# line/Human-Interaction-Generation

Measured on AMD Instinct MI355X. Metric: denoiser-fwd frames/s @ B=64·T=196, higher is better.
Workload: dtype f32; 1 GPU; MotionTransformer forward incl. the per-call cross-attention text side, BASELINE config 2: B=64/GPU T=196 F=150 d=512 L=8 H=8 ff=1024 N=77 Lt=256, linear attention, text embeddings supplied (CLIP stubbed); parallelism=dp1

## Files before the change

### human-interaction-generation_amd/csrc/linattn.hip

```cpp
#include <stdlib.h>

#include "hig_host.h"

namespace {

constexpr int CH = 64;

template <int HD> struct Patch {
  static constexpr int PC = HD >= 128 ? 8 : HD >= 64 ? 4 : HD >= 32 ? 2 : 1;
  static constexpr int PL = PC;
  static constexpr int TL = HD / PL;
};

template <int HD>
__global__ __launch_bounds__(256) void ctx_kernel(const float* __restrict__ K,
                                                  const float* __restrict__ V, int64_t ld, int rows,
                                                  int H, const int64_t* __restrict__ length,
                                                  float* __restrict__ A, float* __restrict__ kstat) {
  constexpr int LDP = HD + 4;
  constexpr int PC = Patch<HD>::PC, PL = Patch<HD>::PL, TL = Patch<HD>::TL;
  constexpr int RG = 256 / HD;
  __shared__ __attribute__((aligned(16))) float sP[CH * LDP];
  __shared__ __attribute__((aligned(16))) float sV[CH * LDP];
  __shared__ float sred[256];
// ... 1388 lines not shown
template <class F> void with_mfma_hd(int hd, F&& f) {
  if (hd == 64) f(std::integral_constant<int, 64>{});
  else f(std::integral_constant<int, 128>{});
}
#define HDC(c) decltype(c)::value

template <typename T> uintptr_t row_bits(int64_t ld) { return hig_low_bits(ld, (int)sizeof(T)); }
template <typename T, class... P> uintptr_t row_bits(int64_t ld, const void* p, P... more) { return hig_low_bits(p) | row_bits<T>(ld, more...); }

}

extern "C" int64_t hig_linattn_ctx_scratch_floats(int32_t B, int32_t rows, int32_t H, int32_t hd) {
  const int64_t nchunk = (rows + CH - 1) / CH;
  return (int64_t)B * H * nchunk * ((int64_t)hd * hd + 2 * hd);
}

namespace {
template <typename TIO>
int launch_ctx(const hig_attn_plan_t& p, const TIO* K, const TIO* V, int64_t ld, int32_t B, int32_t rows, int32_t H, int32_t hd,
               const int64_t* length, float* A, float* kstat, float* scratch, __bf16* At16, hipStream_t st) {
  with_mfma_hd(hd, [&](auto c) {
    if (p.path == HIG_ATTN_PATH_CTX_PART) {
      hipLaunchKernelGGL((ctx_part_mfma_kernel<HDC(c), TIO>), dim3(B * H, p.split), dim3(256), 0, st, K, V, ld, rows, H, length, scratch);
      hipLaunchKernelGGL(ctx_combine_kernel<HDC(c)>, dim3(B * H), dim3(256), 0, st, scratch, p.split, A, kstat, At16);
    } else {
      hipLaunchKernelGGL((ctx_mfma_kernel<HDC(c), TIO>), dim3(B * H), dim3(256), 0, st, K, V, ld, rows, H, length, A, kstat, At16, CtxGroups{H, 0, 0});
    }
  });
  HIG_CHECK_LAUNCH();
  return HIG_OK;
}

template <typename TIO>
int launch_apply(const hig_attn_plan_t& p, const TIO* Q, int64_t ldq, const float* A, TIO* Y, int64_t ldy, int32_t B, int32_t rows, int32_t H,
                 int32_t hd, hipStream_t st) {
  if constexpr (sizeof(TIO) == 4) {
    if (p.path == HIG_ATTN_PATH_APPLY_WAVE64) {
      hipLaunchKernelGGL(apply_wave64_kernel, dim3(B * H), dim3(256), 0, st, reinterpret_cast<const float*>(Q), ldq, A,
                         reinterpret_cast<float*>(Y), ldy, rows, H);
      HIG_CHECK_LAUNCH();
      return HIG_OK;
    }
  }
  with_mfma_hd(hd, [&](auto c) {
    hipLaunchKernelGGL((apply_mfma_kernel<HDC(c), TIO>), dim3(B * H, p.split), dim3(256), 0, st, Q, ldq, A, Y, ldy, rows, H);
  });
  HIG_CHECK_LAUNCH();
  return HIG_OK;
}
}

extern "C" int hig_linattn_ctx(const float* K, const float* V, int64_t ld, int32_t B, int32_t rows,
                               int32_t H, int32_t hd, const int64_t* length, float* A, float* kstat,
                               float* scratch, hig_stream_t stream) {
  hig_attn_plan_t p;
  HIG_TRY(hig_attn_plan_entry(&p, {HIG_ATTN_ENTRY_CTX, HIG_ATTN_IO_F32, B, rows, 0, H, hd, scratch != nullptr, hig_attn_facts(K && V && A && kstat, 0, 0)}));
  if (p.path != HIG_ATTN_PATH_CTX) return launch_ctx<float>(p, K, V, ld, B, rows, H, hd, length, A, kstat, scratch, nullptr, hig_stream(stream));
  HD_SWITCH(hd, hipLaunchKernelGGL((ctx_kernel<HDV>), dim3(B * H), dim3(256), 0, hig_stream(stream), K, V,
                                   ld, rows, H, length, A, kstat));
  HIG_CHECK_LAUNCH();
  return HIG_OK;
}

int hig_linattn_ctx_groups(const float* K, const float* V, int64_t ld, int32_t B, int32_t rows, int32_t H, int32_t G, int32_t hd,
                           float* A, int64_t a_gs, float* kstat, int64_t k_gs, hipStream_t st) {
  if (!hig_attn_mfma_hd(hd) || B <= 0 || rows <= 0 || H <= 0 || G <= 0) return 1;
  with_mfma_hd(hd, [&](auto c) {
    hipLaunchKernelGGL((ctx_mfma_kernel<HDC(c), float>), dim3(B * H * G), dim3(256), 0, st, K, V, ld, rows, H * G, nullptr, A, kstat, nullptr,
                       CtxGroups{H, a_gs, k_gs});
  });
  hig_attn_path_count(HIG_ATTN_PATH_CTX_MFMA, 1);
  HIG_CHECK_LAUNCH();
  return HIG_OK;
}

extern "C" int hig_linattn_apply(const float* Q, int64_t ldq, const float* A, float* Y, int64_t ldy,
                                 int32_t B, int32_t rows, int32_t H, int32_t hd, hig_stream_t stream) {
  hig_attn_plan_t p;
  HIG_TRY(hig_attn_plan_entry(&p, {HIG_ATTN_ENTRY_APPLY, HIG_ATTN_IO_F32, B, rows, 0, H, hd, false,
                     hig_attn_facts(Q && A && Y, row_bits<float>(ldq, Q), row_bits<float>(ldy, Y))}));
  if (p.path != HIG_ATTN_PATH_APPLY) return launch_apply<float>(p, Q, ldq, A, Y, ldy, B, rows, H, hd, hig_stream(stream));
  HD_SWITCH(hd, hipLaunchKernelGGL((apply_kernel<HDV>), dim3(B * H, p.split), dim3(256), 0, hig_stream(stream), Q, ldq, A, Y, ldy, rows, H));
  HIG_CHECK_LAUNCH();
  return HIG_OK;
}

namespace {

template <typename TO> __device__ __forceinline__ float apply_sty_act(float x) { return hig_silu_fast(x); }
template <> __device__ __forceinline__ float apply_sty_act<float>(float x) { return hig_silu(x); }

template <typename T> struct Vec16 {};
template <> struct Vec16<float> { static constexpr int N = 4; };
template <> struct Vec16<__bf16> { static constexpr int N = 8; };
typedef unsigned u32x4_t __attribute__((ext_vector_type(4)));
typedef float f32x4_t __attribute__((ext_vector_type(4)));
__device__ __forceinline__ void put16(float* dst, u32x4_t raw, const float*) {
  *reinterpret_cast<u32x4_t*>(dst) = raw;
}
__device__ __forceinline__ void put16(float* dst, u32x4_t raw, const __bf16*) {
  *reinterpret_cast<f32x4_t*>(dst) = f32x4_t{__uint_as_float(raw.x << 16), __uint_as_float(raw.x & 0xffff0000u),
                                             __uint_as_float(raw.y << 16), __uint_as_float(raw.y & 0xffff0000u)};
  *reinterpret_cast<f32x4_t*>(dst + 4) = f32x4_t{__uint_as_float(raw.z << 16), __uint_as_float(raw.z & 0xffff0000u),
                                                 __uint_as_float(raw.w << 16), __uint_as_float(raw.w & 0xffff0000u)};
}

template <int HD, typename TQ, typename TO>
__global__ __launch_bounds__(256) void apply_sty_kernel(const TQ* __restrict__ Q, int64_t ldq,
                                                        const float* __restrict__ A, const float* __restrict__ gamma,
                                                        const float* __restrict__ beta, const float* __restrict__ ss,
                                                        int64_t ss_ld, int shift_off, TO* __restrict__ Out,
                                                        int64_t ldo, int rows, int H, int nblk) {
  constexpr int TB = HD / 32;
  constexpr int KC = 4096 / HD;
  constexpr int NSLAB = HD / KC;
  constexpr int MAXHPW = 2;
  constexpr int QLD = HD + 4;
  constexpr int EQ = Vec16<TQ>::N;
  constexpr int CPR = HD / EQ;
  constexpr int NQL = 32 * CPR / 64;
  extern __shared__ __attribute__((aligned(16))) char smem_dyn[];
  __shared__ float red[2][4][32];
  const int tid = threadIdx.x, lane = tid & 63, wave = tid >> 6;
  const int lr = lane & 31, kk = lane >> 5;
  const int b = blockIdx.x / nblk, r0 = (blockIdx.x % nblk) * 32;
  const int HPW = H / 4;
  const int d = H * HD;
  constexpr int WBUF = 32 * QLD > KC * HD ? 32 * QLD : KC * HD;
  float* sAw = reinterpret_cast<float*>(smem_dyn) + wave * WBUF;
  float* sQw = sAw;

  f32x16 acc[MAXHPW][TB];
#pragma unroll
  for (int hh = 0; hh < MAXHPW; ++hh)
#pragma unroll
    for (int tb = 0; tb < TB; ++tb) zero16(acc[hh][tb]);

  u32x4_t pq[NQL];
  f32x4_t pa[16];
  auto fetch_q = [&](int h) {
#pragma unroll
    for (int i = 0; i < NQL; ++i) {
      const int idx = lane + 64 * i, rr = idx / CPR, c = idx % CPR;
      const int row = min(r0 + rr, rows - 1);
      pq[i] = *reinterpret_cast<const u32x4_t*>(Q + ((int64_t)b * rows + row) * ldq + h * HD + EQ * c);
    }
  };
  auto fetch_a = [&](int h, int c0) {
    const f32x4_t* src = reinterpret_cast<const f32x4_t*>(A + (((int64_t)b * H + h) * HD + c0) * HD);
#pragma unroll
    for (int i = 0; i < 16; ++i) pa[i] = src[lane + 64 * i];
  };
  fetch_q(wave * HPW);
  fetch_a(wave * HPW, 0);

#pragma unroll
  for (int hh = 0; hh < MAXHPW; ++hh) {
    if (hh >= HPW) break;
    const int h = wave * HPW + hh;
#pragma unroll
    for (int i = 0; i < NQL; ++i) {
      const int idx = lane + 64 * i, rr = idx / CPR, c = idx % CPR;
      put16(sQw + rr * QLD + EQ * c, pq[i], static_cast<const TQ*>(nullptr));
    }
    if (hh + 1 < HPW) fetch_q(h + 1);
    f32x4_t q[HD / 8];
    float m = -INFINITY;
#pragma unroll
    for (int ks = 0; ks < HD / 8; ++ks) {
      q[ks] = *reinterpret_cast<const f32x4_t*>(sQw + lr * QLD + 8 * ks + 4 * kk);
      m = fmaxf(m, fmaxf(fmaxf(q[ks].x, q[ks].y), fmaxf(q[ks].z, q[ks].w)));
    }
    m = fmaxf(m, __shfl_xor(m, 32, 64));
    float sum = 0.f;
#pragma unroll
    for (int ks = 0; ks < HD / 8; ++ks) {
      q[ks].x = __expf(q[ks].x - m); q[ks].y = __expf(q[ks].y - m); q[ks].z = __expf(q[ks].z - m); q[ks].w = __expf(q[ks].w - m);
      sum += (q[ks].x + q[ks].y) + (q[ks].z + q[ks].w);
    }
    sum += __shfl_xor(sum, 32, 64);
    const float inv = 1.0f / sum;
#pragma unroll
    for (int ks = 0; ks < HD / 8; ++ks) q[ks] *= inv;
#pragma unroll
    for (int sl = 0; sl < NSLAB; ++sl) {
      const int c0 = sl * KC;
#pragma unroll
      for (int i = 0; i < 16; ++i) reinterpret_cast<f32x4_t*>(sAw)[lane + 64 * i] = pa[i];
      if (sl + 1 < NSLAB) fetch_a(h, c0 + KC);
      else if (hh + 1 < HPW) fetch_a(h + 1, 0);
#pragma unroll
      for (int ks = c0 / 8; ks < (c0 + KC) / 8; ++ks) {
        const float* ap = sAw + (8 * ks + 4 * kk - c0) * HD + lr;
#pragma unroll
        for (int tb = 0; tb < TB; ++tb)
          acc[hh][tb] = mfma4(acc[hh][tb], ap[32 * tb], ap[HD + 32 * tb], ap[2 * HD + 32 * tb], ap[3 * HD + 32 * tb], make_float4(q[ks].x, q[ks].y, q[ks].z, q[ks].w));
      }
    }
  }
  float s = 0.f;
#pragma unroll
  for (int hh = 0; hh < MAXHPW; ++hh)
#pragma unroll
    for (int tb = 0; tb < TB; ++tb)
#pragma unroll
      for (int e = 0; e < 16; ++e) s += acc[hh][tb][e];
  s += __shfl_xor(s, 32, 64);
  if (kk == 0) red[0][wave][lr] = s;
  __syncthreads();
  const float mean = ((red[0][0][lr] + red[0][1][lr]) + (red[0][2][lr] + red[0][3][lr])) / (float)d;
  float qd = 0.f;
#pragma unroll
  for (int hh = 0; hh < MAXHPW; ++hh) {
    if (hh >= HPW) break;
#pragma unroll
    for (int tb = 0; tb < TB; ++tb)
#pragma unroll
      for (int e = 0; e < 16; ++e) {
        const float dv = acc[hh][tb][e] - mean;
        qd += dv * dv;
      }
  }
  qd += __shfl_xor(qd, 32, 64);
  if (kk == 0) red[1][wave][lr] = qd;
  __syncthreads();
  const float rstd = rsqrtf(((red[1][0][lr] + red[1][1][lr]) + (red[1][2][lr] + red[1][3][lr])) / (float)d + 1e-5f);
  TO* sO = reinterpret_cast<TO*>(smem_dyn);
  const int ldso = d + 16 / (int)sizeof(TO);
  const float* ssrow = ss + (int64_t)b * ss_ld;
#pragma unroll
  for (int hh = 0; hh < MAXHPW; ++hh) {
    if (hh >= HPW) break;
    const int h = wave * HPW + hh;
#pragma unroll
    for (int tb = 0; tb < TB; ++tb)
#pragma unroll
      for (int qq = 0; qq < 4; ++qq) {
        const int col = h * HD + 32 * tb + 8 * qq + 4 * kk;
        const float4 g4 = *reinterpret_cast<const float4*>(gamma + col), b4 = *reinterpret_cast<const float4*>(beta + col);
        const float4 sc = *reinterpret_cast<const float4*>(ssrow + col), sh = *reinterpret_cast<const float4*>(ssrow + shift_off + col);
        float4 o;
        o.x = apply_sty_act<TO>(((acc[hh][tb][4 * qq] - mean) * rstd * g4.x + b4.x) * (1.0f + sc.x) + sh.x);
        o.y = apply_sty_act<TO>(((acc[hh][tb][4 * qq + 1] - mean) * rstd * g4.y + b4.y) * (1.0f + sc.y) + sh.y);
        o.z = apply_sty_act<TO>(((acc[hh][tb][4 * qq + 2] - mean) * rstd * g4.z + b4.z) * (1.0f + sc.z) + sh.z);
        o.w = apply_sty_act<TO>(((acc[hh][tb][4 * qq + 3] - mean) * rstd * g4.w + b4.w) * (1.0f + sc.w) + sh.w);
        st4(sO + lr * ldso + col, o);
      }
  }
  __syncthreads();
  constexpr int EO = 16 / (int)sizeof(TO);
  const int c16 = d / EO;
  for (int idx = tid; idx < 32 * c16; idx += 256) {
    const int rr = idx / c16, ch = idx % c16;
    if (r0 + rr < rows)
      *reinterpret_cast<uint4*>(Out + ((int64_t)b * rows + r0 + rr) * ldo + EO * ch) =
          *reinterpret_cast<const uint4*>(sO + rr * ldso + EO * ch);
  }
}

template <typename TQ, typename TO>
int launch_apply_sty(const TQ* q, int64_t ldq, const float* A, const float* gamma, const float* beta, const float* ss,
                     int64_t ss_ld, int32_t shift_off, TO* o, int64_t ldo, int32_t B, int32_t rows, int32_t H, int32_t hd,
                     hipStream_t st) {
  const int nblk = (rows + 31) / 32;
  const int d = H * hd;
  const size_t wbuf = (size_t)32 * (hd + 4) > 4096 ? (size_t)32 * (hd + 4) : 4096;
  const size_t lds_main = 4 * wbuf * sizeof(float);
  const size_t lds_out = (size_t)32 * (d + 16 / sizeof(TO)) * sizeof(TO);
  const size_t lds = lds_main > lds_out ? lds_main : lds_out;
  constexpr bool HAS64 = !std::is_same<TQ, float>::value;
  static const int big_lds_rc = [] {
    hipError_t e1 = hipSuccess;
    if constexpr (HAS64)
      e1 = hipFuncSetAttribute(reinterpret_cast<const void*>(&apply_sty_kernel<64, TQ, TO>),
                               hipFuncAttributeMaxDynamicSharedMemorySize, 156 * 1024);
    hipError_t e2 = hipFuncSetAttribute(reinterpret_cast<const void*>(&apply_sty_kernel<128, TQ, TO>),
                                        hipFuncAttributeMaxDynamicSharedMemorySize, 156 * 1024);
    return (e1 == hipSuccess && e2 == hipSuccess) ? 0 : 1;
  }();
  if (big_lds_rc != 0 || lds > 156 * 1024)
    return hig_set_error(HIG_EHIP, "hig_linattn_apply_sty: cannot reserve %zu bytes of LDS", lds);
  if (hd == 64) {
    if constexpr (HAS64)
      hipLaunchKernelGGL((apply_sty_kernel<64, TQ, TO>), dim3(B * nblk), dim3(256), lds, st, q, ldq, A, gamma, beta, ss, ss_ld,
                         shift_off, o, ldo, rows, H, nblk);
    else
      return hig_set_error(HIG_EUNSUPPORTED, "hig_linattn_apply_sty: head dim 64 has its own fp32 kernel");
  } else
    hipLaunchKernelGGL((apply_sty_kernel<128, TQ, TO>), dim3(B * nblk), dim3(256), lds, st, q, ldq, A, gamma, beta, ss, ss_ld,
                       shift_off, o, ldo, rows, H, nblk);
  HIG_CHECK_LAUNCH();
  return HIG_OK;
}

template <int H>
__global__ __launch_bounds__(64 * H, 4) void apply_sty_wave64_kernel(const float* __restrict__ Q, int64_t ldq, const float* __restrict__ A,
                                                                    const float* __restrict__ gamma, const float* __restrict__ beta,
                                                                    const float* __restrict__ ss, int64_t ss_ld, int shift_off,
                                                                    float* __restrict__ Out, int64_t ldo, int rows) {
  constexpr int HD = 64, D = H * HD;
  __shared__ __attribute__((aligned(16))) float sW[H * 16 * HD];
  __shared__ __attribute__((aligned(16))) float sP[4 * D];
  __shared__ float2 sR[2][H][16];
  const int tid = threadIdx.x, lane = tid & 63, h = tid >> 6;
  const int b = blockIdx.x;
  const int r = lane & 15, kq = lane >> 4;
  const int ntile = (rows + 15) >> 4, step = gridDim.y;
  const float* qb = Q + (int64_t)b * rows * ldq + h * HD + 16 * kq;
  la_f32x4 qt[4];
  auto fetch = [&](int tile, la_f32x4 (&v)[4]) {
    const int row = min(min(tile, ntile - 1) * 16 + r, rows - 1);
    const float* p = qb + (int64_t)row * ldq;
    asm volatile("global_load_dwordx4 %0, %4, off\n\tglobal_load_dwordx4 %1, %4, off offset:16\n\t"
                 "global_load_dwordx4 %2, %4, off offset:32\n\tglobal_load_dwordx4 %3, %4, off offset:48"
                 : "=&v"(v[0]), "=&v"(v[1]), "=&v"(v[2]), "=&v"(v[3]) : "v"(p) : "memory");
  };
  int tile = blockIdx.y;
  fetch(tile, qt);
  float aop[16][4];
  {
    const float4* Ab = reinterpret_cast<const float4*>(A + (((int64_t)b * H + h) * HD + 16 * kq) * HD) + r;
#pragma unroll
    for (int s2 = 0; s2 < 16; ++s2) {
      const float4 a4 = Ab[s2 * (HD / 4)];
      aop[s2][0] = a4.x; aop[s2][1] = a4.y; aop[s2][2] = a4.z; aop[s2][3] = a4.w;
    }
    const int arr = tid / (D / 4), idx = tid % (D / 4);
    const float* ssrow = ss + (int64_t)b * ss_ld;
    const float* src = arr == 0 ? gamma : arr == 1 ? beta : arr == 2 ? ssrow : ssrow + shift_off;
    float4 pv = *reinterpret_cast<const float4*>(src + 4 * idx);
    if (arr == 2) pv = make_float4(1.0f + pv.x, 1.0f + pv.y, 1.0f + pv.z, 1.0f + pv.w);
    *reinterpret_cast<float4*>(sP + arr * D + 4 * idx) = pv;
  }
  float* const so = sW + h * (16 * HD);
  __syncthreads();
  [[maybe_unused]] __amdgpu_buffer_rsrc_t rsO = __builtin_amdgcn_make_buffer_rsrc(Out + (int64_t)b * rows * ldo, 0, (int)(((int64_t)(rows - 1) * ldo + D) * 4), 0x00020000);
  int par = 0;
  auto tile_out = [&](int tile, auto younger) {
    la_f32x4 (&cur)[4] = qt;
    constexpr int YOUNGER = decltype(younger)::value;
    asm volatile("s_waitcnt vmcnt(%4)" : "+v"(cur[0]), "+v"(cur[1]), "+v"(cur[2]), "+v"(cur[3]) : "n"(YOUNGER) : "memory");
    float m = fmaxf(fmaxf(fmaxf(cur[0].x, cur[0].y), fmaxf(cur[0].z, cur[0].w)), fmaxf(fmaxf(cur[1].x, cur[1].y), fmaxf(cur[1].z, cur[1].w)));
    m = fmaxf(m, fmaxf(fmaxf(fmaxf(cur[2].x, cur[2].y), fmaxf(cur[2].z, cur[2].w)), fmaxf(fmaxf(cur[3].x, cur[3].y), fmaxf(cur[3].z, cur[3].w))));
    m = fmaxf(m, __shfl_xor(m, 16, 64));
    m = fmaxf(m, __shfl_xor(m, 32, 64));
    float p[16];
    float sum = 0.f;
#pragma unroll
    for (int i = 0; i < 4; ++i) {
      p[4 * i] = __expf(cur[i].x - m); p[4 * i + 1] = __expf(cur[i].y - m); p[4 * i + 2] = __expf(cur[i].z - m); p[4 * i + 3] = __expf(cur[i].w - m);
      sum += (p[4 * i] + p[4 * i + 1]) + (p[4 * i + 2] + p[4 * i + 3]);
    }
    sum += __shfl_xor(sum, 16, 64);
    sum += __shfl_xor(sum, 32, 64);
    const float inv = 1.0f / sum;
    la_f32x4 acc[4];
#pragma unroll
    for (int blk = 0; blk < 4; ++blk) acc[blk] = la_f32x4{0.f, 0.f, 0.f, 0.f};
#pragma unroll
    for (int s2 = 0; s2 < 16; ++s2) {
      const float ps = p[s2] * inv;
#pragma unroll
      for (int blk = 0; blk < 4; ++blk) acc[blk] = __builtin_amdgcn_mfma_f32_16x16x4f32(aop[s2][blk], ps, acc[blk], 0, 0, 0);
    }
    float bs = 0.f;
#pragma unroll
    for (int blk = 0; blk < 4; ++blk) bs += (acc[blk][0] + acc[blk][1]) + (acc[blk][2] + acc[blk][3]);
    bs += __shfl_xor(bs, 16, 64);
    bs += __shfl_xor(bs, 32, 64);
    const float bm = bs * (1.0f / HD);
    float bq = 0.f;
#pragma unroll
    for (int blk = 0; blk < 4; ++blk) {
      const float d0 = acc[blk][0] - bm, d1 = acc[blk][1] - bm, d2 = acc[blk][2] - bm, d3 = acc[blk][3] - bm;
      bq += (d0 * d0 + d1 * d1) + (d2 * d2 + d3 * d3);
    }
    bq += __shfl_xor(bq, 16, 64);
    bq += __shfl_xor(bq, 32, 64);
#pragma unroll
    for (int e = 0; e < 4; ++e)
      *reinterpret_cast<la_f32x4*>(so + r * HD + ((16 * kq + 4 * e) ^ (4 * r))) = la_f32x4{acc[0][e], acc[1][e], acc[2][e], acc[3][e]};
    if (kq == 0) sR[par][h][r] = make_float2(bs, bq);
    lds_barrier();
    float tot = 0.f, within = 0.f;
#pragma unroll
    for (int hh = 0; hh < H; ++hh) {
      const float2 ps = sR[par][hh][r];
      tot += ps.x; within += ps.y;
    }
    const float mean = tot * (1.0f / D);
    asm volatile("" ::: "memory");
    float between = 0.f;
#pragma unroll
    for (int hh = 0; hh < H; ++hh) {
      const float dm = fmaf(sR[par][hh][r].x, 1.0f / HD, -mean);
      between = fmaf(dm, dm, between);
    }
    par ^= 1;
    const float rstd = rsqrtf(fmaf((float)HD, between, within) * (1.0f / D) + 1e-5f);
#pragma unroll
    for (int e = 0; e < 4; ++e) {
      const int col = h * HD + 16 * kq + 4 * e;
      const float4 g4 = *reinterpret_cast<const float4*>(sP + col), b4 = *reinterpret_cast<const float4*>(sP + D + col);
      const float4 sc = *reinterpret_cast<const float4*>(sP + 2 * D + col), sh = *reinterpret_cast<const float4*>(sP + 3 * D + col);
      float* const yp = so + r * HD + ((16 * kq + 4 * e) ^ (4 * r));
      const float4 y4 = *reinterpret_cast<const float4*>(yp);
      float4 o;
      o.x = hig_silu(((y4.x - mean) * rstd * g4.x + b4.x) * sc.x + sh.x);
      o.y = hig_silu(((y4.y - mean) * rstd * g4.y + b4.y) * sc.y + sh.y);
      o.z = hig_silu(((y4.z - mean) * rstd * g4.z + b4.z) * sc.z + sh.z);
      o.w = hig_silu(((y4.w - mean) * rstd * g4.w + b4.w) * sc.w + sh.w);
      *reinterpret_cast<float4*>(yp) = o;
      asm volatile("" ::: "memory");
    }
    fetch(tile + step < ntile ? tile + step : tile, qt);
    asm volatile("s_waitcnt lgkmcnt(0)" ::: "memory");
#pragma unroll
    for (int i = 0; i < 4; ++i) {
      const int rr = 4 * i + kq, cc = 4 * r;
      [[maybe_unused]] const float4 v = *reinterpret_cast<const float4*>(so + rr * HD + (cc ^ (4 * rr)));
      [[maybe_unused]] const int row = tile * 16 + rr;
#if defined(__HIP_DEVICE_COMPILE__)
      __builtin_amdgcn_raw_buffer_store_b128(__builtin_bit_cast(la_i32x4, v), rsO, (row * (int)ldo + h * HD + cc) * 4, 0, 0);
#endif
    }
    asm volatile("s_waitcnt lgkmcnt(0)" ::: "memory");
  };
  tile_out(tile, std::integral_constant<int, 0>{});
  for (tile += step; tile < ntile; tile += step) tile_out(tile, std::integral_constant<int, 4>{});
  asm volatile("s_waitcnt vmcnt(0)" ::: "memory");
}

template <int H>
int launch_apply_sty_wave64(const float* q, int64_t ldq, const float* A, const float* gamma, const float* beta, const float* ss,
                            int64_t ss_ld, int32_t shift_off, float* o, int64_t ldo, int32_t B, int32_t rows, int nstrip, hipStream_t st) {
  hipLaunchKernelGGL((apply_sty_wave64_kernel<H>), dim3(B, nstrip), dim3(64 * H), 0, st, q, ldq, A, gamma, beta, ss, ss_ld, shift_off, o,
                     ldo, rows);
  HIG_CHECK_LAUNCH();
  return HIG_OK;
}

template <typename TIO>
int launch_apply_bwd(const hig_attn_plan_t& p, const TIO* dY, int64_t lddy, const TIO* Q, int64_t ldq, const float* A, TIO* dQ, int64_t lddq,
                     float* dA, int32_t B, int32_t rows, int32_t H, int32_t hd, float* scratch, hipStream_t st) {
  const bool merge = p.variant & HIG_ATTN_VARIANT_MERGE;
  if (p.path == HIG_ATTN_PATH_APPLY_BWD_MFMA) {
    with_mfma_hd(hd, [&](auto c) {
      hipLaunchKernelGGL((apply_bwd_mfma_kernel<HDC(c), TIO>), dim3(B * H, p.split), dim3(256), attn_bwd_lds_bytes<HDC(c)>(), st, dY, lddy, Q,
                         ldq, A, dQ, lddq, merge ? scratch : dA, rows, H);
    });
  } else if constexpr (sizeof(TIO) == 4) {
    HD_SWITCH(hd, hipLaunchKernelGGL((apply_bwd_kernel<HDV>), dim3(B * H, p.split), dim3(256), 0, st, dY, lddy, Q, ldq, A, dQ, lddq, scratch,
                                     rows, H));
  }
  HIG_CHECK_LAUNCH();
  if (!merge) return HIG_OK;
  const int64_t n = (int64_t)hd * hd, groups = (int64_t)B * H;
  const int64_t want = (groups * n / 4 + 255) / 256;
  hipLaunchKernelGGL(chunk_sum_kernel, dim3((unsigned)(want > 2048 ? 2048 : want)), dim3(256), 0, st, scratch, p.split, n, groups, dA);
  HIG_CHECK_LAUNCH();
  return HIG_OK;
}

template <typename TIO>
int launch_ctx_bwd(const hig_attn_plan_t& p, const float* dA, const float* A, const TIO* K, const TIO* V, int64_t ld, const float* kstat,
                   const int64_t* length, TIO* dK, TIO* dV, int64_t ldd, int32_t B, int32_t rows, int32_t H, int32_t hd, float* scratch,
                   hipStream_t st) {
  if (p.path == HIG_ATTN_PATH_CTX_BWD_MFMA) {
    with_mfma_hd(hd, [&](auto c) {
      hipLaunchKernelGGL((ctx_bwd_mfma_kernel<HDC(c), TIO>), dim3(B * H, p.split), dim3(256), attn_bwd_lds_bytes<HDC(c)>(), st, dA, A, K, V, ld,
                         kstat, length, dK, dV, ldd, rows, H);
    });
  } else if constexpr (sizeof(TIO) == 4) {
    HD_SWITCH(hd, hipLaunchKernelGGL((ctx_bwd_kernel<HDV>), dim3(B * H, p.split), dim3(256), 0, st, dA, K, V, ld, kstat, length, dK, dV, ldd,
                                     rows, H, scratch));
    HIG_CHECK_LAUNCH();
    HD_SWITCH(hd, hipLaunchKernelGGL((ctx_bwd_finish_kernel<HDV>), dim3(B * H, p.split), dim3(256), 0, st, K, ld, kstat, length, dK, ldd, rows,
                                     H, scratch));
  }
  HIG_CHECK_LAUNCH();
  return HIG_OK;
}

int plan_bwd_entry(hig_attn_plan_t* p, const hig_attn_call& c) {
  hig_attn_call aligned = c;
  aligned.facts |= HIG_ATTN_FACT_IN8 | HIG_ATTN_FACT_IN16 | HIG_ATTN_FACT_OUT8 | HIG_ATTN_FACT_OUT16;
  const bool would_use = c.hd == 128 && hig_attn_plan_for(aligned, hig_attn_switch_values(), hig_chip_cus(), true).rc == HIG_OK;
  return hig_attn_plan_entry(p, c, !would_use || allow_big_lds() == 0);
}
bool sty_out_i32(int64_t rows, int64_t ldo) { return rows <= 0 || ldo <= (INT32_MAX / 4) / (rows + 16); }

}

extern "C" int hig_linattn_ctx_bf16(const void* K, const void* V, int64_t ld, int32_t B, int32_t rows, int32_t H,
                                    int32_t hd, const int64_t* length, float* A, float* kstat, float* scratch,
                                    void* At16, hig_stream_t stream) {
  hig_attn_plan_t p;
  HIG_TRY(hig_attn_plan_entry(&p, {HIG_ATTN_ENTRY_CTX, HIG_ATTN_IO_BF16, B, rows, 0, H, hd, scratch != nullptr,
                              hig_attn_facts(K && V && A && kstat, row_bits<__bf16>(ld, K, V), 0)}));
  return launch_ctx<__bf16>(p, static_cast<const __bf16*>(K), static_cast<const __bf16*>(V), ld, B, rows, H, hd, length, A, kstat, scratch,
                            static_cast<__bf16*>(At16), hig_stream(stream));
}
extern "C" int hig_linattn_apply_bf16(const void* Q, int64_t ldq, const float* A, void* Y, int64_t ldy, int32_t B,
                                      int32_t rows, int32_t H, int32_t hd, hig_stream_t stream) {
  hig_attn_plan_t p;
  HIG_TRY(hig_attn_plan_entry(&p, {HIG_ATTN_ENTRY_APPLY, HIG_ATTN_IO_BF16, B, rows, 0, H, hd, false,
                              hig_attn_facts(Q && A && Y, row_bits<__bf16>(ldq, Q), row_bits<__bf16>(ldy, Y))}));
  return launch_apply<__bf16>(p, static_cast<const __bf16*>(Q), ldq, A, static_cast<__bf16*>(Y), ldy, B, rows, H, hd, hig_stream(stream));
}

extern "C" int64_t hig_linattn_bwd_scratch_floats(int32_t B, int32_t rows, int32_t H, int32_t hd) {
  const int64_t nchunk = (rows + CH - 1) / CH;
  return (int64_t)B * H * nchunk * ((int64_t)hd * hd + hd);
}

extern "C" int hig_linattn_apply_bwd(const float* dY, int64_t lddy, const float* Q, int64_t ldq,
                                     const float* A, float* dQ, int64_t lddq, float* dA, int32_t B,
                                     int32_t rows, int32_t H, int32_t hd, float* scratch,
                                     hig_stream_t stream) {
  hig_attn_plan_t p;
  HIG_TRY(plan_bwd_entry(&p, {HIG_ATTN_ENTRY_APPLY_BWD, HIG_ATTN_IO_F32, B, rows, 0, H, hd, scratch != nullptr,
                              hig_attn_facts(dY && Q && A && dQ && dA, row_bits<float>(ldq, Q) | row_bits<float>(lddy, dY), row_bits<float>(lddq, dQ))}));
  return launch_apply_bwd<float>(p, dY, lddy, Q, ldq, A, dQ, lddq, dA, B, rows, H, hd, scratch, hig_stream(stream));
}

extern "C" int hig_linattn_ctx_bwd(const float* dA, const float* A, const float* K, const float* V, int64_t ld,
                                   const float* kstat, const int64_t* length, float* dK, float* dV,
                                   int64_t ldd, int32_t B, int32_t rows, int32_t H, int32_t hd,
                                   float* scratch, hig_stream_t stream) {
  hig_attn_plan_t p;
  HIG_TRY(plan_bwd_entry(&p, {HIG_ATTN_ENTRY_CTX_BWD, HIG_ATTN_IO_F32, B, rows, 0, H, hd, scratch != nullptr,
                              hig_attn_facts(dA && A && K && V && kstat && dK && dV, 0, row_bits<float>(ldd, dK, dV))}));
  return launch_ctx_bwd<float>(p, dA, A, K, V, ld, kstat, length, dK, dV, ldd, B, rows, H, hd, scratch, hig_stream(stream));
}

extern "C" int hig_linattn_apply_bwd_bf16(const void* dY, int64_t lddy, const void* Q, int64_t ldq, const float* A, void* dQ,
                                          int64_t lddq, float* dA, int32_t B, int32_t rows, int32_t H, int32_t hd, float* scratch,
                                          hig_stream_t stream) {
  hig_attn_plan_t p;
  HIG_TRY(plan_bwd_entry(&p, {HIG_ATTN_ENTRY_APPLY_BWD, HIG_ATTN_IO_BF16, B, rows, 0, H, hd, scratch != nullptr,
                              hig_attn_facts(dY && Q && A && dQ && dA, row_bits<__bf16>(ldq, Q) | row_bits<__bf16>(lddy, dY), row_bits<__bf16>(lddq, dQ))}));
  return launch_apply_bwd<__bf16>(p, static_cast<const __bf16*>(dY), lddy, static_cast<const __bf16*>(Q), ldq, A, static_cast<__bf16*>(dQ), lddq,
                                  dA, B, rows, H, hd, scratch, hig_stream(stream));
}
extern "C" int hig_linattn_ctx_bwd_bf16(const float* dA, const float* A, const void* K, const void* V, int64_t ld, const float* kstat,
                                        const int64_t* length, void* dK, void* dV, int64_t ldd, int32_t B, int32_t rows, int32_t H,
                                        int32_t hd, hig_stream_t stream) {
  hig_attn_plan_t p;
  HIG_TRY(plan_bwd_entry(&p, {HIG_ATTN_ENTRY_CTX_BWD, HIG_ATTN_IO_BF16, B, rows, 0, H, hd, false,
                              hig_attn_facts(dA && A && K && V && kstat && dK && dV, row_bits<__bf16>(ld, K, V), row_bits<__bf16>(ldd, dK, dV))}));
  return launch_ctx_bwd<__bf16>(p, dA, A, static_cast<const __bf16*>(K), static_cast<const __bf16*>(V), ld, kstat, length,
                                static_cast<__bf16*>(dK), static_cast<__bf16*>(dV), ldd, B, rows, H, hd, nullptr, hig_stream(stream));
}

extern "C" int hig_linattn_apply_sty_bf16(const void* Q, int64_t ldq, const float* A, const float* gamma,
                                          const float* beta, const float* ss, int64_t ss_ld, int32_t ss_shift_off,
                                          void* Out, int64_t ldo, int32_t B, int32_t rows, int32_t H, int32_t hd,
                                          hig_stream_t stream) {
  hig_attn_plan_t p;
  HIG_TRY(hig_attn_plan_entry(&p, {HIG_ATTN_ENTRY_APPLY_STY, HIG_ATTN_IO_BF16, B, rows, 0, H, hd, false,
                              hig_attn_facts(Q && A && gamma && beta && ss && Out, row_bits<__bf16>(ldq, Q), row_bits<__bf16>(ldo, Out),
                                             row_bits<float>(ss_ld, gamma, beta, ss) | row_bits<float>(ss_shift_off))}));
  return launch_apply_sty<__bf16, __bf16>(static_cast<const __bf16*>(Q), ldq, A, gamma, beta, ss, ss_ld, ss_shift_off,
                                          static_cast<__bf16*>(Out), ldo, B, rows, H, hd, hig_stream(stream));
}

extern "C" int hig_linattn_apply_sty(const float* Q, int64_t ldq, const float* A, const float* gamma, const float* beta,
                                     const float* ss, int64_t ss_ld, int32_t ss_shift_off, float* Out, int64_t ldo,
                                     int32_t B, int32_t rows, int32_t H, int32_t hd, hig_stream_t stream) {
  hig_attn_plan_t p;
  HIG_TRY(hig_attn_plan_entry(&p, {HIG_ATTN_ENTRY_APPLY_STY, HIG_ATTN_IO_F32, B, rows, 0, H, hd, false,
                              hig_attn_facts(Q && A && gamma && beta && ss && Out, row_bits<float>(ldq, Q), row_bits<float>(ldo, Out),
                                             row_bits<float>(ss_ld, gamma, beta, ss) | row_bits<float>(ss_shift_off),
                                             sty_out_i32(rows, ldo))}));
  if (p.path == HIG_ATTN_PATH_APPLY_STY)
    return launch_apply_sty<float, float>(Q, ldq, A, gamma, beta, ss, ss_ld, ss_shift_off, Out, ldo, B, rows, H, hd, hig_stream(stream));
  return H == 8 ? launch_apply_sty_wave64<8>(Q, ldq, A, gamma, beta, ss, ss_ld, ss_shift_off, Out, ldo, B, rows, p.split, hig_stream(stream))
                : launch_apply_sty_wave64<4>(Q, ldq, A, gamma, beta, ss, ss_ld, ss_shift_off, Out, ldo, B, rows, p.split, hig_stream(stream));
}

static long long g_attn_launches[HIG_ATTN_NPATHS];
static int g_attn_last_split = 1;
void hig_attn_path_count(int path, int split) {
  if (path < 0 || path >= HIG_ATTN_NPATHS) return;
  __atomic_fetch_add(&g_attn_launches[path], 1, __ATOMIC_RELAXED);
  __atomic_store_n(&g_attn_last_split, split, __ATOMIC_RELAXED);
}
extern "C" int64_t hig_attn_path_launches(int32_t path) {
  if (path < 0 || path >= HIG_ATTN_NPATHS) return -1;
  return __atomic_load_n(&g_attn_launches[path], __ATOMIC_RELAXED);
}
extern "C" int32_t hig_attn_last_split(void) { return __atomic_load_n(&g_attn_last_split, __ATOMIC_RELAXED); }
```

Before: 2.148 million frames/s.

## Prefetch Q tiles straight into LDS with buffer loads in wave64 apply kernel

In the head-dim-64 styled apply kernel, the next Q tile is now prefetched with `buffer_load ... lds` directly into a per-wave shared-memory slot, and read back from LDS, instead of being fetched into registers at the end of each tile. The gamma/beta/scale/shift parameter load is issued earlier. Its store to shared memory is deferred into the first tile's body after the MFMA chain, and the block-wide barrier is removed. This aims to hide global latency for Q and shorten the kernel prologue. It costs extra LDS, depends on a hand-written M0 swizzle, and relies on later synchronisation to make the parameter writes visible to other waves.

```diff
diff --git a/human-interaction-generation_amd/csrc/linattn.hip b/human-interaction-generation_amd/csrc/linattn.hip
--- a/human-interaction-generation_amd/csrc/linattn.hip
+++ b/human-interaction-generation_amd/csrc/linattn.hip
@@ -1714,11 +1714,38 @@
   __shared__ __attribute__((aligned(16))) float sW[H * 16 * HD];
   __shared__ __attribute__((aligned(16))) float sP[4 * D];
   __shared__ float2 sR[2][H][16];
+  __shared__ __attribute__((aligned(16))) float sQ[H * 16 * HD];
   const int tid = threadIdx.x, lane = tid & 63, h = tid >> 6;
   const int b = blockIdx.x;
   const int r = lane & 15, kq = lane >> 4;
   const int ntile = (rows + 15) >> 4, step = gridDim.y;
   const float* qb = Q + (int64_t)b * rows * ldq + h * HD + 16 * kq;
+  const int hu = __builtin_amdgcn_readfirstlane(h);
+  float* const sq = sQ + hu * (16 * HD);
+  [[maybe_unused]] const unsigned sq_lds = (unsigned)(size_t)(__attribute__((address_space(3))) float*)sQ + (unsigned)hu * (16 * HD * 4);
+  [[maybe_unused]] la_i32x4 rsQ;
+  {
+    const uint64_t qa = (uint64_t)(Q + (int64_t)b * rows * ldq);
+    rsQ = la_i32x4{(int)(uint32_t)qa, (int)(uint32_t)((qa >> 32) & 0xffffu), (int)(((int64_t)(rows - 1) * ldq + D) * 4), 0x00020000};
+  }
+  const int qcol = (hu * HD) * 4 + 16 * (r ^ kq);
+  auto prefetch = [&](int tile) {
+    [[maybe_unused]] int vo[4];
+#pragma unroll
+    for (int n = 0; n < 4; ++n) vo[n] = min(tile * 16 + 4 * n + kq, rows - 1) * ((int)ldq * 4) + (qcol ^ (64 * n));
+#if defined(__HIP_DEVICE_COMPILE__)
+    unsigned keep;
+    asm volatile("s_mov_b32 %0, m0\n\t"
+                 "s_mov_b32 m0, %6\n\ts_nop 0\n\tbuffer_load_dwordx4 %1, %5, 0 offen lds\n\t"
+                 "s_mov_b32 m0, %7\n\ts_nop 0\n\tbuffer_load_dwordx4 %2, %5, 0 offen lds\n\t"
+                 "s_mov_b32 m0, %8\n\ts_nop 0\n\tbuffer_load_dwordx4 %3, %5, 0 offen lds\n\t"
+                 "s_mov_b32 m0, %9\n\ts_nop 0\n\tbuffer_load_dwordx4 %4, %5, 0 offen lds\n\t"
+                 "s_mov_b32 m0, %0"
+                 : "=&s"(keep)
+                 : "v"(vo[0]), "v"(vo[1]), "v"(vo[2]), "v"(vo[3]), "s"(rsQ), "s"(sq_lds), "s"(sq_lds + 1024u), "s"(sq_lds + 2048u), "s"(sq_lds + 3072u)
+                 : "memory");
+#endif
+  };
   la_f32x4 qt[4];
   auto fetch = [&](int tile, la_f32x4 (&v)[4]) {
     const int row = min(min(tile, ntile - 1) * 16 + r, rows - 1);
@@ -1728,6 +1755,13 @@
                  : "=&v"(v[0]), "=&v"(v[1]), "=&v"(v[2]), "=&v"(v[3]) : "v"(p) : "memory");
   };
   int tile = blockIdx.y;
+  const int arr = tid / (D / 4), idx = tid % (D / 4);
+  float4 pv;
+  {
+    const float* ssrow = ss + (int64_t)b * ss_ld;
+    const float* src = arr == 0 ? gamma : arr == 1 ? beta : arr == 2 ? ssrow : ssrow + shift_off;
+    pv = *reinterpret_cast<const float4*>(src + 4 * idx);
+  }
   fetch(tile, qt);
   float aop[16][4];
   {
@@ -1737,21 +1771,21 @@
       const float4 a4 = Ab[s2 * (HD / 4)];
       aop[s2][0] = a4.x; aop[s2][1] = a4.y; aop[s2][2] = a4.z; aop[s2][3] = a4.w;
     }
-    const int arr = tid / (D / 4), idx = tid % (D / 4);
-    const float* ssrow = ss + (int64_t)b * ss_ld;
-    const float* src = arr == 0 ? gamma : arr == 1 ? beta : arr == 2 ? ssrow : ssrow + shift_off;
-    float4 pv = *reinterpret_cast<const float4*>(src + 4 * idx);
-    if (arr == 2) pv = make_float4(1.0f + pv.x, 1.0f + pv.y, 1.0f + pv.z, 1.0f + pv.w);
-    *reinterpret_cast<float4*>(sP + arr * D + 4 * idx) = pv;
   }
   float* const so = sW + h * (16 * HD);
-  __syncthreads();
   [[maybe_unused]] __amdgpu_buffer_rsrc_t rsO = __builtin_amdgcn_make_buffer_rsrc(Out + (int64_t)b * rows * ldo, 0, (int)(((int64_t)(rows - 1) * ldo + D) * 4), 0x00020000);
   int par = 0;
-  auto tile_out = [&](int tile, auto younger) {
+  auto tile_out = [&](int tile, auto first) {
     la_f32x4 (&cur)[4] = qt;
-    constexpr int YOUNGER = decltype(younger)::value;
-    asm volatile("s_waitcnt vmcnt(%4)" : "+v"(cur[0]), "+v"(cur[1]), "+v"(cur[2]), "+v"(cur[3]) : "n"(YOUNGER) : "memory");
+    if constexpr (decltype(first)::value) {
+      asm volatile("s_waitcnt vmcnt(16)" : "+v"(cur[0]), "+v"(cur[1]), "+v"(cur[2]), "+v"(cur[3]) : : "memory");
+    } else {
+      asm volatile("s_waitcnt vmcnt(4)" ::: "memory");
+#pragma unroll
+      for (int i = 0; i < 4; ++i) cur[i] = *reinterpret_cast<const la_f32x4*>(sq + r * HD + ((16 * kq + 4 * i) ^ (4 * r)));
+      asm volatile("s_waitcnt lgkmcnt(0)" : "+v"(cur[0]), "+v"(cur[1]), "+v"(cur[2]), "+v"(cur[3]) : : "memory");
+      if (tile + step < ntile) prefetch(tile + step);
+    }
     float m = fmaxf(fmaxf(fmaxf(cur[0].x, cur[0].y), fmaxf(cur[0].z, cur[0].w)), fmaxf(fmaxf(cur[1].x, cur[1].y), fmaxf(cur[1].z, cur[1].w)));
     m = fmaxf(m, fmaxf(fmaxf(fmaxf(cur[2].x, cur[2].y), fmaxf(cur[2].z, cur[2].w)), fmaxf(fmaxf(cur[3].x, cur[3].y), fmaxf(cur[3].z, cur[3].w))));
     m = fmaxf(m, __shfl_xor(m, 16, 64));
@@ -1774,6 +1808,11 @@
       const float ps = p[s2] * inv;
 #pragma unroll
       for (int blk = 0; blk < 4; ++blk) acc[blk] = __builtin_amdgcn_mfma_f32_16x16x4f32(aop[s2][blk], ps, acc[blk], 0, 0, 0);
+    }
+    if constexpr (decltype(first)::value) {
+      if (arr == 2) pv = make_float4(1.0f + pv.x, 1.0f + pv.y, 1.0f + pv.z, 1.0f + pv.w);
+      *reinterpret_cast<float4*>(sP + arr * D + 4 * idx) = pv;
+      if (tile + step < ntile) prefetch(tile + step);
     }
     float bs = 0.f;
 #pragma unroll
@@ -1825,7 +1864,6 @@
       *reinterpret_cast<float4*>(yp) = o;
       asm volatile("" ::: "memory");
     }
-    fetch(tile + step < ntile ? tile + step : tile, qt);
     asm volatile("s_waitcnt lgkmcnt(0)" ::: "memory");
 #pragma unroll
     for (int i = 0; i < 4; ++i) {
@@ -1838,9 +1876,8 @@
     }
     asm volatile("s_waitcnt lgkmcnt(0)" ::: "memory");
   };
-  tile_out(tile, std::integral_constant<int, 0>{});
-  for (tile += step; tile < ntile; tile += step) tile_out(tile, std::integral_constant<int, 4>{});
-  asm volatile("s_waitcnt vmcnt(0)" ::: "memory");
+  tile_out(tile, std::true_type{});
+  for (tile += step; tile < ntile; tile += step) tile_out(tile, std::false_type{});
 }
 
 template <int H>
```

Result: no change. 2.162 million frames/s (median of 6 runs) (+0.6%).
